# microsoft/MoGe

Measured on AMD Instinct MI355X. Metric: images/sec (MoGeModel.infer, moge-2-vitl 518x518 fp16), higher is better.
Workload: dtype f16; 1 GPU; moge-2-vitl infer(): batch 32/GPU x 3x518x518 torch.rand, num_tokens 3600, fp16 weights, synthetic checkpoint (seed 0), inputs resident in HBM, outputs left on device; global_batch=32, parallelism=dp1 (independent shards, one-time RCCL weight broadcast)

## Files before the change

moge_amd/csrc/attention_pp.hip:

```cpp
#include "common.h"

#define AP_GPTR(p) ((const __attribute__((address_space(1))) void*)(p))
#define AP_LPTR(p) ((__attribute__((address_space(3))) void*)(p))

typedef short s16x4 __attribute__((ext_vector_type(4)));

__device__ __forceinline__ u32x4 tr_pair(const char* p0, const char* p1) {
    const s16x4 a = __builtin_amdgcn_ds_read_tr16_b64_v4i16((__attribute__((address_space(3))) s16x4*)(p0));
    const s16x4 b = __builtin_amdgcn_ds_read_tr16_b64_v4i16((__attribute__((address_space(3))) s16x4*)(p1));
    typedef short s16x8 __attribute__((ext_vector_type(8)));
    const s16x8 v = {a[0], a[1], a[2], a[3], b[0], b[1], b[2], b[3]};
    return __builtin_bit_cast(u32x4, v);
}

__device__ __forceinline__ u32x4 pack8(const f32x16& p, int s) {
    f16x8 h;
#pragma unroll
    for (int i = 0; i < 8; i++) h[i] = (f16)p[8 * s + i];
    return __builtin_bit_cast(u32x4, h);
}

constexpr int AP_STAGE = 16384;
constexpr float AP_PSUM_LIMIT = 16384.f;

#ifdef MOGE_EXPERIMENTS
#include "../../tools/experiments/attention_pp_exp.inc"
#endif

constexpr int AP_VAR_DEFAULT = 0;
constexpr int AP_X_DEFAULT = 0;
constexpr int AP_KERN_DEFAULT = 3;
constexpr float AP_SCORE_LIMIT = 15.f;
constexpr float AP_ROWSUM_LIMIT = 49152.f;
template <int VAR>
__global__ __launch_bounds__(256, 3) void attn_pp16_kernel(const f16* __restrict__ q, const f16* __restrict__ k, const f16* __restrict__ v,
                                                           f16* __restrict__ out, int Ntok, int nh) {
    constexpr int NW = 4, NPW = 4;
    extern __shared__ __attribute__((aligned(16))) char smem[];

    const int tid = threadIdx.x, lane = tid & 63;
    const int wave = __builtin_amdgcn_readfirstlane(tid >> 6);
    const int l15 = lane & 15, g4 = lane >> 4;
    const int bh = blockIdx.y;
    const int b = bh / nh, head = bh - b * nh;
    const int q0 = blockIdx.x * (NW * 32) + wave * 32;

    u32x4 qf[2][2];
#pragma unroll
    for (int qb = 0; qb < 2; qb++) {
        const int qrow = q0 + qb * 16 + l15;
        const f16* qp = q + ((size_t)bh * Ntok + (qrow < Ntok ? qrow : Ntok - 1)) * 64;
#pragma unroll
        for (int ks = 0; ks < 2; ks++) qf[qb][ks] = *reinterpret_cast<const u32x4*>(qp + 32 * ks + 8 * g4);
    }

    const char* kbase = reinterpret_cast<const char*>(k + (size_t)bh * Ntok * 64);
    const char* vbase = reinterpret_cast<const char*>(v + (size_t)bh * Ntok * 64);
    const int prow = lane >> 3, pch = lane & 7;
    int drow[NPW];
    unsigned doff[NPW];
#pragma unroll
    for (int i = 0; i < NPW; i++) {
        const int p = wave + NW * i;
        const int row = (p & 7) * 8 + prow;
        drow[i] = row;
        const int ksw = ((row >> 1) & 1) | (((row >> 3) & 3) << 1);
        const int vsw = (((row >> 1) & 1) << 1) | (((row >> 3) & 1) << 2);
        doff[i] = (unsigned)(row * 128 + ((pch ^ (p >= 8 ? vsw : ksw)) << 4));
    }
    const int ntiles = (Ntok + 63) >> 6;
    auto issue = [&](int t) {
        char* st = smem + (t % 3) * AP_STAGE;
        const char* kt = uniform_ptr(kbase + (size_t)t * 8192);
        const char* vt = uniform_ptr(vbase + (size_t)t * 8192);
        if (t < ntiles - 1) {
#pragma unroll
            for (int i = 0; i < NPW; i++) {
                const int p = wave + NW * i;
                __builtin_amdgcn_global_load_lds(AP_GPTR((p >= 8 ? vt : kt) + doff[i]), AP_LPTR(st + p * 1024), 16, 0, 0);
            }
        } else {
#pragma unroll
            for (int i = 0; i < NPW; i++) {
                const int p = wave + NW * i;
                const int over = t * 64 + drow[i] - (Ntok - 1);
                const unsigned off = doff[i] - (over > 0 ? (unsigned)over * 128u : 0u);
                __builtin_amdgcn_global_load_lds(AP_GPTR((p >= 8 ? vt : kt) + off), AP_LPTR(st + p * 1024), 16, 0, 0);
            }
        }
    };

    const int kswl = ((l15 >> 1) & 1) | ((l15 >> 2) << 1);
    int kaddr[2];
#pragma unroll
    for (int ks = 0; ks < 2; ks++) kaddr[ks] = (8 * (l15 >> 2) + (l15 & 3)) * 128 + (((4 * ks + g4) ^ kswl) << 4);
    const int vswl = (((l15 >> 3) & 1) << 1) | ((g4 & 1) << 2);
    int vaddr[4];
#pragma unroll
    for (int db = 0; db < 4; db++)
        vaddr[db] = 8192 + (8 * g4 + (l15 >> 2)) * 128 + ((((2 * db) ^ vswl) | ((l15 & 3) >> 1)) << 4) + (l15 & 1) * 8;

    f32x4 o[4][2];
    f32x4 negs[2];
    float m_run[2], l_run[2];
#pragma unroll
    for (int qb = 0; qb < 2; qb++) {
#pragma unroll
        for (int db = 0; db < 4; db++) o[db][qb] = f32x4{0.f, 0.f, 0.f, 0.f};
        negs[qb] = f32x4{0.f, 0.f, 0.f, 0.f};
        m_run[qb] = -1e30f; l_run[qb] = 0.f;
    }

    issue(0);
    if (ntiles > 1) issue(1);

    int stage = 0;
    const char* ka[2];
    const char* va[4];
    f32x4 sc[4][2];
    float psum[2];
    auto tile_head = [&](int t) {
        if (t + 1 < ntiles) asm volatile("s_waitcnt vmcnt(%0)" ::"n"(NPW) : "memory");
        else asm volatile("s_waitcnt vmcnt(0)" ::: "memory");
        __builtin_amdgcn_s_barrier();
        asm volatile("" ::: "memory");
        if (t + 2 < ntiles) issue(t + 2);
        const int so = stage * AP_STAGE;
        stage = stage == 2 ? 0 : stage + 1;
#pragma unroll
        for (int ks = 0; ks < 2; ks++) ka[ks] = smem + (kaddr[ks] + so);
#pragma unroll
        for (int db = 0; db < 4; db++) va[db] = smem + (vaddr[db] + so);
    };
    auto pv = [&]() {
#pragma unroll
        for (int qb = 0; qb < 2; qb++) l_run[qb] += psum[qb];
#pragma unroll
        for (int s2 = 0; s2 < 2; s2++) {
            u32x4 pf[2];
#pragma unroll
            for (int qb = 0; qb < 2; qb++) {
                f16x8 hp;
#pragma unroll
                for (int r = 0; r < 4; r++) { hp[r] = (f16)sc[2 * s2][qb][r]; hp[4 + r] = (f16)sc[2 * s2 + 1][qb][r]; }
                pf[qb] = __builtin_bit_cast(u32x4, hp);
            }
#pragma unroll
            for (int db = 0; db < 4; db++) {
                const u32x4 vf = tr_pair(va[db] + (32 * ((VAR & 32) ? 0 : s2)) * 128, va[db] + (32 * ((VAR & 32) ? 0 : s2) + 4) * 128);
#pragma unroll
                for (int qb = 0; qb < 2; qb++) mma16<f16>(o[db][qb], vf, pf[qb]);
            }
        }
    };
    auto exact_body = [&](int t, bool last) {
#pragma unroll
        for (int kb = 0; kb < 4; kb++) {
            const int koff = (32 * (kb >> 1) + 4 * (kb & 1)) * 128;
            const u32x4 kf0 = *reinterpret_cast<const u32x4*>(ka[0] + koff), kf1 = *reinterpret_cast<const u32x4*>(ka[1] + koff);
#pragma unroll
            for (int qb = 0; qb < 2; qb++) {
                sc[kb][qb] = f32x4{0.f, 0.f, 0.f, 0.f};
                mma16<f16>(sc[kb][qb], kf0, qf[qb][0]);
                mma16<f16>(sc[kb][qb], kf1, qf[qb][1]);
            }
        }
#pragma unroll
        for (int qb = 0; qb < 2; qb++) {
            if (last) {
#pragma unroll
                for (int kb = 0; kb < 4; kb++)
#pragma unroll
                    for (int r = 0; r < 4; r++) {
                        const int key = t * 64 + 32 * (kb >> 1) + 8 * g4 + 4 * (kb & 1) + r;
                        if (key >= Ntok) sc[kb][qb][r] = -1e30f;
                    }
            }
            float mx = sc[0][qb][0];
#pragma unroll
            for (int kb = 0; kb < 4; kb++)
#pragma unroll
                for (int r = 0; r < 4; r++) mx = fmaxf(mx, sc[kb][qb][r]);
            mx = fmaxf(mx, __shfl_xor(mx, 16));
            mx = fmaxf(mx, __shfl_xor(mx, 32));
            const float m_new = fmaxf(m_run[qb], mx);
            const float alpha = __builtin_amdgcn_exp2f(m_run[qb] - m_new);
            m_run[qb] = m_new;
            l_run[qb] *= alpha;
#pragma unroll
            for (int db = 0; db < 4; db++)
#pragma unroll
                for (int r = 0; r < 4; r++) o[db][qb][r] *= alpha;
#pragma unroll
            for (int r = 0; r < 4; r++) negs[qb][r] = -m_new;
            float ps = 0.f;
#pragma unroll
            for (int kb = 0; kb < 4; kb++)
#pragma unroll
                for (int r = 0; r < 4; r++) {
                    sc[kb][qb][r] = __builtin_amdgcn_exp2f(sc[kb][qb][r] - m_new);
                    ps += sc[kb][qb][r];
                }
            psum[qb] = ps;
        }
        pv();
    };

    tile_head(0);
    exact_body(0, ntiles == 1);
    int t = 1;
    for (;;) {
        bool hit = false;
        for (; t < ntiles - 1; t++) {
            tile_head(t);
            if constexpr (VAR & 4) {
                u32x4 kf[4][2];
#pragma unroll
                for (int kb = 0; kb < 4; kb++) {
                    const int koff = (32 * (kb >> 1) + 4 * (kb & 1)) * 128;
                    kf[kb][0] = *reinterpret_cast<const u32x4*>(ka[0] + koff);
                    kf[kb][1] = *reinterpret_cast<const u32x4*>(ka[1] + koff);
                }
#pragma unroll
                for (int kb = 0; kb < 4; kb++)
#pragma unroll
                    for (int qb = 0; qb < 2; qb++)
                        sc[kb][qb] = __builtin_amdgcn_mfma_f32_16x16x32_f16(__builtin_bit_cast(f16x8, kf[kb][0]), __builtin_bit_cast(f16x8, qf[qb][0]), negs[qb], 0, 0, 0);
#pragma unroll
                for (int kb = 0; kb < 4; kb++)
#pragma unroll
                    for (int qb = 0; qb < 2; qb++) mma16<f16>(sc[kb][qb], kf[kb][1], qf[qb][1]);
            } else {
#pragma unroll
            for (int kb = 0; kb < 4; kb++) {
                const int koff = (32 * (kb >> 1) + 4 * (kb & 1)) * 128;
                const u32x4 kf0 = *reinterpret_cast<const u32x4*>(ka[0] + koff), kf1 = *reinterpret_cast<const u32x4*>(ka[1] + koff);
#pragma unroll
                for (int qb = 0; qb < 2; qb++) {
                    sc[kb][qb] = __builtin_amdgcn_mfma_f32_16x16x32_f16(__builtin_bit_cast(f16x8, kf0), __builtin_bit_cast(f16x8, qf[qb][0]), negs[qb], 0, 0, 0);
                    mma16<f16>(sc[kb][qb], kf1, qf[qb][1]);
                }
            }
            }
            bool trig = false;
            if constexpr ((VAR & 8) != 0) {
                float mx = sc[0][0][0];
#pragma unroll
                for (int kb = 0; kb < 4; kb++)
#pragma unroll
                    for (int qb = 0; qb < 2; qb++)
#pragma unroll
                        for (int r = 0; r < 4; r++) mx = fmaxf(mx, sc[kb][qb][r]);
                trig = !(mx <= AP_SCORE_LIMIT);
                if (__builtin_expect(__any(trig), 0)) { hit = true; break; }
            }
#pragma unroll
            for (int qb = 0; qb < 2; qb++) {
                float ps0 = 0.f, ps1 = 0.f;
#pragma unroll
                for (int kb = 0; kb < 4; kb++)
#pragma unroll
                    for (int r = 0; r < 4; r++) {
                        sc[kb][qb][r] = (VAR & 1) ? sc[kb][qb][r] * 1e-3f : __builtin_amdgcn_exp2f(sc[kb][qb][r]);
                        if (!(VAR & 16) || (kb == 0 && r == 0)) { if (kb & 1) ps1 += sc[kb][qb][r]; else ps0 += sc[kb][qb][r]; }
                    }
                psum[qb] = ps0 + ps1;
                trig |= !(psum[qb] < AP_PSUM_LIMIT);
            }
            if constexpr ((VAR & (2 | 8)) == 0) {
                if (__builtin_expect(__any(trig), 0)) { hit = true; break; }
            }
            pv();
        }
        if (!hit) break;
        exact_body(t, false);
        t++;
    }
    if (ntiles > 1) {
        tile_head(ntiles - 1);
        exact_body(ntiles - 1, true);
    }
#pragma unroll
    for (int qb = 0; qb < 2; qb++) {
        float l_tot = l_run[qb] + __shfl_xor(l_run[qb], 16);
        l_tot += __shfl_xor(l_tot, 32);
        const float inv = 1.f / l_tot;
        const int qrow = q0 + qb * 16 + l15;
        if (qrow < Ntok) {
            f16* op = out + ((size_t)b * Ntok + qrow) * ((size_t)nh * 64) + head * 64;
#pragma unroll
            for (int db = 0; db < 4; db++)
                store4(op + 16 * db + 4 * g4, o[db][qb][0] * inv, o[db][qb][1] * inv, o[db][qb][2] * inv, o[db][qb][3] * inv);
        }
    }
}

template <int QB> struct AttnAcc { f32x4 o[4][QB]; float m[QB], l[QB]; };
template <int QB, bool SK = false>
__device__ __forceinline__ bool attn_pp16mq_body(const f16* __restrict__ q, const f16* __restrict__ k, const f16* __restrict__ v, f16* __restrict__ out,
                                                 int Ntok, int nh, int bh, int q_base, char* smem, int tb_in = 0, int te_in = 0, AttnAcc<QB>* acc = nullptr,
                                                 const char* seed_k = nullptr) {
    constexpr int NW = 4, NPW = 4;
    const int tid = threadIdx.x, lane = tid & 63;
    const int wave = __builtin_amdgcn_readfirstlane(tid >> 6) & (NW - 1);
    const int l15 = lane & 15, g4 = lane >> 4;
    const int b = bh / nh, head = bh - b * nh;
    const int q0 = q_base + wave * (16 * QB);
    u32x4 qf[QB][2];
#pragma unroll
    for (int qb = 0; qb < QB; qb++) {
        const int qrow = q0 + qb * 16 + l15;
        const f16* qp = q + ((size_t)bh * Ntok + (qrow < Ntok ? qrow : Ntok - 1)) * 64;
#pragma unroll
        for (int ks = 0; ks < 2; ks++) qf[qb][ks] = *reinterpret_cast<const u32x4*>(qp + 32 * ks + 8 * g4);
    }
    const char* kbase = reinterpret_cast<const char*>(k + (size_t)bh * Ntok * 64);
    const char* vbase = reinterpret_cast<const char*>(v + (size_t)bh * Ntok * 64);
    const int prow = lane >> 3, pch = lane & 7;
    unsigned doff[NPW], doff_last[NPW];
    const int ntiles = (Ntok + 63) >> 6;
    const int tb = SK ? tb_in : 0, te = SK ? te_in : ntiles;
#pragma unroll
    for (int i = 0; i < NPW; i++) {
        const int p = wave + NW * i;
        const int row = (p & 7) * 8 + prow;
        const int ksw = ((row >> 1) & 1) | (((row >> 3) & 3) << 1);
        const int vsw = (((row >> 1) & 1) << 1) | (((row >> 3) & 1) << 2);
        doff[i] = (unsigned)(row * 128 + ((pch ^ (p >= 8 ? vsw : ksw)) << 4));
        const int over = (ntiles - 1) * 64 + row - (Ntok - 1);
        doff_last[i] = doff[i] - (over > 0 ? (unsigned)over * 128u : 0u);
    }
    auto issue = [&](int t) {
        char* st = smem + ((SK ? t - tb : t) % 3) * AP_STAGE;
        const char* kt = uniform_ptr(kbase + (size_t)t * 8192);
        const char* vt = uniform_ptr(vbase + (size_t)t * 8192);
        const bool last = t >= ntiles - 1;
#pragma unroll
        for (int i = 0; i < NPW; i++) {
            const int p = wave + NW * i;
            __builtin_amdgcn_global_load_lds(AP_GPTR((p >= 8 ? vt : kt) + (last ? doff_last[i] : doff[i])), AP_LPTR(st + p * 1024), 16, 0, 0);
        }
    };
    const int kswl = ((l15 >> 1) & 1) | ((l15 >> 2) << 1);
    int kaddr[2];
#pragma unroll
    for (int ks = 0; ks < 2; ks++) kaddr[ks] = (8 * (l15 >> 2) + (l15 & 3)) * 128 + (((4 * ks + g4) ^ kswl) << 4);
    const int vswl = (((l15 >> 3) & 1) << 1) | ((g4 & 1) << 2);
    int vaddr[4];
#pragma unroll
    for (int db = 0; db < 4; db++)
        vaddr[db] = 8192 + (8 * g4 + (l15 >> 2)) * 128 + ((((2 * db) ^ vswl) | ((l15 & 3) >> 1)) << 4) + (l15 & 1) * 8;

    f32x4 o[4][QB];
    f32x4 negs[QB];
    float m_run[QB], l_run[QB];
#pragma unroll
    for (int qb = 0; qb < QB; qb++) {
#pragma unroll
        for (int db = 0; db < 4; db++) o[db][qb] = f32x4{0.f, 0.f, 0.f, 0.f};
        negs[qb] = f32x4{0.f, 0.f, 0.f, 0.f};
        m_run[qb] = -1e30f; l_run[qb] = 0.f;
    }
    issue(tb);
    if (te - tb > 1) issue(tb + 1);

    int stage = 0;
    const char* ka[2];
    const char* va[4];
    f32x4 sc[4][QB];
    float psum[QB];
    auto tile_head = [&](int t, bool with_issue = true) {
        if (t + 1 < te) asm volatile("s_waitcnt vmcnt(%0)" ::"n"(NPW) : "memory");
        else asm volatile("s_waitcnt vmcnt(0)" ::: "memory");
        __builtin_amdgcn_s_barrier();
        asm volatile("" ::: "memory");
        if (with_issue && t + 2 < te) issue(t + 2);
        const int so = stage * AP_STAGE;
        stage = stage == 2 ? 0 : stage + 1;
#pragma unroll
        for (int ks = 0; ks < 2; ks++) ka[ks] = smem + (kaddr[ks] + so);
#pragma unroll
        for (int db = 0; db < 4; db++) va[db] = smem + (vaddr[db] + so);
    };
    auto pack = [&](int qb, u32x4 (&pf)[2]) {
#pragma unroll
        for (int s2 = 0; s2 < 2; s2++) {
            f16x8 hp;
#pragma unroll
            for (int r = 0; r < 4; r++) { hp[r] = (f16)sc[2 * s2][qb][r]; hp[4 + r] = (f16)sc[2 * s2 + 1][qb][r]; }
            pf[s2] = __builtin_bit_cast(u32x4, hp);
        }
    };
    auto pv_block = [&](int qb, const u32x4 (&pf)[2]) {
        l_run[qb] += psum[qb];
#pragma unroll
        for (int s2 = 0; s2 < 2; s2++)
#pragma unroll
            for (int db = 0; db < 4; db++) {
                const u32x4 vf = tr_pair(va[db] + (32 * s2) * 128, va[db] + (32 * s2 + 4) * 128);
                mma16<f16>(o[db][qb], vf, pf[s2]);
            }
    };
    auto exact_block = [&](int t, bool last, int qb) {
#pragma unroll
        for (int kb = 0; kb < 4; kb++) {
            const int koff = (32 * (kb >> 1) + 4 * (kb & 1)) * 128;
            const u32x4 kf0 = *reinterpret_cast<const u32x4*>(ka[0] + koff), kf1 = *reinterpret_cast<const u32x4*>(ka[1] + koff);
            sc[kb][qb] = f32x4{0.f, 0.f, 0.f, 0.f};
            mma16<f16>(sc[kb][qb], kf0, qf[qb][0]);
            mma16<f16>(sc[kb][qb], kf1, qf[qb][1]);
        }
        if (last) {
#pragma unroll
            for (int kb = 0; kb < 4; kb++)
#pragma unroll
                for (int r = 0; r < 4; r++) {
                    const int key = t * 64 + 32 * (kb >> 1) + 8 * g4 + 4 * (kb & 1) + r;
                    if (key >= Ntok) sc[kb][qb][r] = -1e30f;
                }
        }
        float mx = sc[0][qb][0];
#pragma unroll
        for (int kb = 0; kb < 4; kb++)
#pragma unroll
            for (int r = 0; r < 4; r++) mx = fmaxf(mx, sc[kb][qb][r]);
        mx = fmaxf(mx, __shfl_xor(mx, 16));
        mx = fmaxf(mx, __shfl_xor(mx, 32));
        const float m_new = fmaxf(m_run[qb], mx);
        const float alpha = __builtin_amdgcn_exp2f(m_run[qb] - m_new);
        m_run[qb] = m_new;
        l_run[qb] *= alpha;
#pragma unroll
        for (int db = 0; db < 4; db++)
#pragma unroll
            for (int r = 0; r < 4; r++) o[db][qb][r] *= alpha;
#pragma unroll
        for (int r = 0; r < 4; r++) negs[qb][r] = -m_new;
        float ps = 0.f;
#pragma unroll
        for (int kb = 0; kb < 4; kb++)
#pragma unroll
            for (int r = 0; r < 4; r++) {
                sc[kb][qb][r] = __builtin_amdgcn_exp2f(sc[kb][qb][r] - m_new);
                ps += sc[kb][qb][r];
            }
        ps += __shfl_xor(ps, 16);
        ps += __shfl_xor(ps, 32);
        psum[qb] = ps;
        u32x4 pf[2];
        pack(qb, pf);
        pv_block(qb, pf);
    };
    auto qk_block = [&](int qb, const u32x4 (&kf)[4][2]) {
#pragma unroll
        for (int kb = 0; kb < 4; kb++)
            sc[kb][qb] = __builtin_amdgcn_mfma_f32_16x16x32_f16(__builtin_bit_cast(f16x8, kf[kb][0]), __builtin_bit_cast(f16x8, qf[qb][0]), negs[qb], 0, 0, 0);
#pragma unroll
        for (int kb = 0; kb < 4; kb++) mma16<f16>(sc[kb][qb], kf[kb][1], qf[qb][1]);
    };
    u32x4 ones;
#pragma unroll
    for (int i = 0; i < 4; i++) ones[i] = 0x3c003c00u;
    const f32x4 zero4 = {0.f, 0.f, 0.f, 0.f};

    if (__builtin_amdgcn_readfirstlane(q0) >= Ntok) {
        for (int tt = tb; tt < te; tt++) tile_head(tt);
        return false;
    }
    bool seeded = false;
    if constexpr (SK) seeded = seed_k != nullptr && tb < ntiles - 1;
    tile_head(tb, !seeded);
    if constexpr (SK) if (seed_k) {
#pragma unroll
        for (int qb = 0; qb < QB; qb++) {
            float mx = -1e30f;
#pragma unroll
            for (int kb = 0; kb < 4; kb++) {
                const int koff = (32 * (kb >> 1) + 4 * (kb & 1)) * 128;
                const u32x4 kf0 = *reinterpret_cast<const u32x4*>(seed_k + kaddr[0] + koff), kf1 = *reinterpret_cast<const u32x4*>(seed_k + kaddr[1] + koff);
                f32x4 s0 = {0.f, 0.f, 0.f, 0.f};
                mma16<f16>(s0, kf0, qf[qb][0]);
                mma16<f16>(s0, kf1, qf[qb][1]);
#pragma unroll
                for (int r = 0; r < 4; r++) mx = fmaxf(mx, s0[r]);
            }
            mx = fmaxf(mx, __shfl_xor(mx, 16));
            mx = fmaxf(mx, __shfl_xor(mx, 32));
            m_run[qb] = mx;
#pragma unroll
            for (int r = 0; r < 4; r++) negs[qb][r] = -mx;
        }
    }
    int t = tb + 1;
    if (seeded) t = tb;
    else {
#pragma unroll
        for (int qb = 0; qb < QB; qb++) exact_block(tb, tb == ntiles - 1, qb);
    }
    const int hot_end = SK ? (te < ntiles - 1 ? te : ntiles - 1) : ntiles - 1;
    u32x4 pf[QB][2];
    f32x4 lt[QB];
    for (;;) {
        bool hit = false;
        for (; t < hot_end; t++) {
            if (!(seeded && t == tb)) tile_head(t, false);
            u32x4 kf[4][2];
#pragma unroll
            for (int kb = 0; kb < 4; kb++) {
                const int koff = (32 * (kb >> 1) + 4 * (kb & 1)) * 128;
                kf[kb][0] = *reinterpret_cast<const u32x4*>(ka[0] + koff);
                kf[kb][1] = *reinterpret_cast<const u32x4*>(ka[1] + koff);
            }
            __builtin_amdgcn_sched_barrier(0);
            if (t + 2 < te) issue(t + 2);
            __builtin_amdgcn_sched_barrier(0);
#pragma unroll
            for (int qb = 0; qb < QB; qb++) qk_block(qb, kf);
#pragma unroll
            for (int qb = 0; qb < QB; qb++) {
#pragma unroll
                for (int kb = 0; kb < 4; kb++)
#pragma unroll
                    for (int r = 0; r < 4; r++) sc[kb][qb][r] = __builtin_amdgcn_exp2f(sc[kb][qb][r]);
                pack(qb, pf[qb]);
                lt[qb] = __builtin_amdgcn_mfma_f32_16x16x32_f16(__builtin_bit_cast(f16x8, ones), __builtin_bit_cast(f16x8, pf[qb][0]), zero4, 0, 0, 0);
                mma16<f16>(lt[qb], ones, pf[qb][1]);
            }
            bool trig = false;
#pragma unroll
            for (int qb = 0; qb < QB; qb++) trig |= !(lt[qb][0] < AP_ROWSUM_LIMIT);
            if (__builtin_expect(__any(trig), 0)) { hit = true; break; }
#pragma unroll
            for (int qb = 0; qb < QB; qb++) l_run[qb] += lt[qb][0];
            {
                constexpr int AHEAD = QB == 4 ? 5 : 4;
                u32x4 vf[8];
                auto ld = [&](int gi) { vf[gi] = tr_pair(va[gi & 3] + (32 * (gi >> 2)) * 128, va[gi & 3] + (32 * (gi >> 2) + 4) * 128); };
#pragma unroll
                for (int gi = 0; gi < AHEAD; gi++) ld(gi);
                __builtin_amdgcn_sched_barrier(0);
#pragma unroll
                for (int gi = 0; gi < 8; gi++) {
                    if (gi + AHEAD < 8) ld(gi + AHEAD);
#pragma unroll
                    for (int qb = 0; qb < QB; qb++) mma16<f16>(o[gi & 3][qb], vf[gi], pf[qb][gi >> 2]);
                    __builtin_amdgcn_sched_barrier(0);
                }
            }
        }
        if (!hit) break;
#pragma unroll
        for (int qb = 0; qb < QB; qb++) {
            if (__any(!(lt[qb][0] < AP_ROWSUM_LIMIT))) exact_block(t, false, qb);
            else { psum[qb] = lt[qb][0]; pv_block(qb, pf[qb]); }
        }
        t++;
    }
    if (SK ? (te == ntiles && ntiles - 1 > tb) : (ntiles > 1)) {
        tile_head(ntiles - 1);
#pragma unroll
        for (int qb = 0; qb < QB; qb++) exact_block(ntiles - 1, true, qb);
    }
    if constexpr (SK) {
#pragma unroll
        for (int qb = 0; qb < QB; qb++) {
#pragma unroll
            for (int db = 0; db < 4; db++) acc->o[db][qb] = o[db][qb];
            acc->m[qb] = m_run[qb]; acc->l[qb] = l_run[qb];
        }
        return true;
    }
#pragma unroll
    for (int qb = 0; qb < QB; qb++) {
        const float inv = 1.f / l_run[qb];
        const int qrow = q0 + qb * 16 + l15;
        if (qrow < Ntok) {
            f16* op = out + ((size_t)b * Ntok + qrow) * ((size_t)nh * 64) + head * 64;
#pragma unroll
            for (int db = 0; db < 4; db++)
                store4(op + 16 * db + 4 * g4, o[db][qb][0] * inv, o[db][qb][1] * inv, o[db][qb][2] * inv, o[db][qb][3] * inv);
        }
    }
    return true;
}

template <int QB>
__global__ __launch_bounds__(256, QB > 2 ? 2 : 3) void attn_pp16mq_kernel(const f16* __restrict__ q, const f16* __restrict__ k, const f16* __restrict__ v,
                                                            f16* __restrict__ out, int Ntok, int nh, int xcd_remap, int q_start) {
    extern __shared__ __attribute__((aligned(16))) char smem[];
    int bh = blockIdx.y, qblk = blockIdx.x;
    if (((gridDim.y & 7) == 0) && (xcd_remap & 1)) {
        const int lin = blockIdx.y * gridDim.x + blockIdx.x;
        const int x = lin & 7, s = lin >> 3;
        const int hs = s / (int)gridDim.x;
        bh = x + 8 * hs;
        qblk = s - hs * (int)gridDim.x;
    }
    const int q_base = q_start + qblk * (64 * QB);
    if constexpr (QB == 4) if (xcd_remap & 2) {
        if (Ntok - q_base <= 128) { attn_pp16mq_body<2>(q, k, v, out, Ntok, nh, bh, q_base, smem); return; }
    }
    attn_pp16mq_body<QB>(q, k, v, out, Ntok, nh, bh, q_base, smem);
}

constexpr int AP_KS_MIN_TILES = 8;
template <int QB>
__global__ __launch_bounds__(512, 1) void attn_pp16ks_kernel(const f16* __restrict__ q, const f16* __restrict__ k, const f16* __restrict__ v,
                                                            f16* __restrict__ out, int Ntok, int nh, int xcd_remap, int tmid) {
    extern __shared__ __attribute__((aligned(16))) char smem[];
    int bh = blockIdx.y, qblk = blockIdx.x;
    if (((gridDim.y & 7) == 0) && (xcd_remap & 1)) {
        const int lin = blockIdx.y * gridDim.x + blockIdx.x;
        const int x = lin & 7, s = lin >> 3;
        const int hs = s / (int)gridDim.x;
        bh = x + 8 * hs;
        qblk = s - hs * (int)gridDim.x;
    }
    const int q_base = qblk * (64 * QB);
    const int tid = threadIdx.x, lane = tid & 63, t4 = tid & 255;
    const int wave8 = __builtin_amdgcn_readfirstlane(tid >> 6), grp = wave8 >> 2, wave = wave8 & 3;
    const int ntiles = (Ntok + 63) >> 6;
    AttnAcc<QB> a;
    const bool active = attn_pp16mq_body<QB, true>(q, k, v, out, Ntok, nh, bh, q_base, smem + grp * (3 * AP_STAGE), grp ? tmid : 0, grp ? ntiles : tmid, &a, grp ? smem : nullptr);
    for (int i = grp ? ntiles - tmid : tmid, n = max(tmid, ntiles - tmid); i < n; i++) __builtin_amdgcn_s_barrier();
    __syncthreads();
    f32x4* ex_o = reinterpret_cast<f32x4*>(smem);
    f32x2* ex_ml = reinterpret_cast<f32x2*>(smem + (size_t)4 * QB * 256 * 16);
    if (grp && active) {
#pragma unroll
        for (int db = 0; db < 4; db++)
#pragma unroll
            for (int qb = 0; qb < QB; qb++) ex_o[(db * QB + qb) * 256 + t4] = a.o[db][qb];
#pragma unroll
        for (int qb = 0; qb < QB; qb++) ex_ml[qb * 256 + t4] = f32x2{a.m[qb], a.l[qb]};
    }
    __syncthreads();
    if (grp || !active) return;
    const int l15 = lane & 15, g4 = lane >> 4;
    const int b = bh / nh, head = bh - b * nh;
    const int q0 = q_base + wave * (16 * QB);
#pragma unroll
    for (int qb = 0; qb < QB; qb++) {
        const f32x2 ml = ex_ml[qb * 256 + t4];
        const float mstar = fmaxf(a.m[qb], ml[0]);
        const float w0 = __builtin_amdgcn_exp2f(a.m[qb] - mstar), w1 = __builtin_amdgcn_exp2f(ml[0] - mstar);
        const float l = fmaf(w1, ml[1], w0 * a.l[qb]);
        const float inv = 1.f / l;
        const int qrow = q0 + qb * 16 + l15;
#pragma unroll
        for (int db = 0; db < 4; db++) {
            const f32x4 o1 = ex_o[(db * QB + qb) * 256 + t4];
            f32x4 o;
#pragma unroll
            for (int r = 0; r < 4; r++) o[r] = fmaf(w1, o1[r], w0 * a.o[db][qb][r]);
            if (qrow < Ntok) {
                f16* op = out + ((size_t)b * Ntok + qrow) * ((size_t)nh * 64) + head * 64;
                store4(op + 16 * db + 4 * g4, o[0] * inv, o[1] * inv, o[2] * inv, o[3] * inv);
            }
        }
    }
}

#ifdef MOGE_EXPERIMENTS
#include "../../tools/experiments/attention_pp16sk_exp.inc"
#else
size_t attention_pp_ws_bytes(int, int, int) { return 0; }
size_t attention_pp_ws_counter_bytes(int, int, int) { return 0; }
#endif

#ifdef MOGE_EXPERIMENTS
#include "../../tools/experiments/attention_pp16s_exp.inc"
#include "../../tools/experiments/attention_pp16x_exp.inc"
#endif


static int launch_attn_pp16(const void* q, const void* k, const void* v, void* out, int B, int nh, int Ntok, hipStream_t st, void* ws, size_t ws_bytes) {
    constexpr int smem = 3 * AP_STAGE;
#ifdef MOGE_EXPERIMENTS
    {
        int QB, nx, gx;
        if (ws && attn_sk_plan(B, nh, Ntok, &QB, &nx, &gx) && ws_bytes >= attention_pp_ws_bytes(B, nh, Ntok)) {
            int* cnt = reinterpret_cast<int*>(ws);
            float* part = reinterpret_cast<float*>(reinterpret_cast<char*>(ws) + attention_pp_ws_counter_bytes(B, nh, Ntok));
            if (QB == 4) {
                if (int rc = set_dyn_lds<attn_pp16sk_kernel<4>>(smem)) return rc;
                hipLaunchKernelGGL(attn_pp16sk_kernel<4>, dim3(nx * gx), dim3(256), smem, st, (const f16*)q, (const f16*)k, (const f16*)v, (f16*)out, Ntok, nh, nx, B * nh / nx, part, cnt);
            } else {
                if (int rc = set_dyn_lds<attn_pp16sk_kernel<2>>(smem)) return rc;
                hipLaunchKernelGGL(attn_pp16sk_kernel<2>, dim3(nx * gx), dim3(256), smem, st, (const f16*)q, (const f16*)k, (const f16*)v, (f16*)out, Ntok, nh, nx, B * nh / nx, part, cnt);
            }
            return (int)hipGetLastError();
        }
    }
#else
    (void)ws; (void)ws_bytes;
#endif
    dim3 grid((Ntok + 127) / 128, B * nh);
    const int akern = moge_tune_get("ATTN_KERN", AP_KERN_DEFAULT);
    if (akern >= 1) {
        const long wgs2 = (long)((Ntok + 127) / 128) * B * nh;
        const bool q4 = akern == 2 || akern == 4 || (akern == 3 && wgs2 > moge_tune_get("ATTN_Q2_MAX_WGS", 3 * pp_device_cus()));
        const int xr = (moge_tune_get("ATTN_XCD", 1) ? 1 : 0) | (moge_tune_get("ATTN_TAIL2", 1) ? 2 : 0);
#ifdef MOGE_EXPERIMENTS
        const int nfull = Ntok / 512, rem = Ntok - nfull * 512;
        const int nblk = nfull + (rem > 256 ? 1 : 0);
        const bool xk = nblk > 0 && (akern == 4 || (akern == 3 && moge_tune_get("ATTN_X", AP_X_DEFAULT) &&
                                                    (long)nblk * B * nh >= (long)moge_tune_get("ATTN_X_MIN_ROUNDS", 2) * pp_device_cus()));
        if (xk) {
            constexpr int smem_x = 4 * AP_STAGE + 8 * 8192;
            if (moge_tune_get("ATTN_X_TS", 0)) {
                static unsigned long long* dts = nullptr;
                if (!dts && hipMalloc(&dts, 16 * sizeof(unsigned long long)) != hipSuccess) return -1;
                (void)hipMemsetAsync(dts, 0, 16 * sizeof(unsigned long long), st);
                if (int rc = set_dyn_lds<attn_pp16x_kernel<0, 1>>(smem_x)) return rc;
                hipLaunchKernelGGL((attn_pp16x_kernel<0, 1>), dim3(nblk, B * nh), dim3(512), smem_x, st, (const f16*)q, (const f16*)k, (const f16*)v, (f16*)out, Ntok, nh, xr, dts);
                unsigned long long h[16];
                (void)hipMemcpyAsync(h, dts, sizeof(h), hipMemcpyDeviceToHost, st);
                (void)hipStreamSynchronize(st);
                for (int g2 = 0; g2 < 2; g2++)
                    if (h[g2 * 8 + 4])
                        fprintf(stderr, "[attn_pp16x ts] group %d: %llu hot tiles; per tile (s_memtime ticks): E body %.0f, barrier wait %.0f, M body %.0f, barrier wait %.0f\n", g2, h[g2 * 8 + 4],
                                (double)h[g2 * 8 + 0] / h[g2 * 8 + 4], (double)h[g2 * 8 + 1] / h[g2 * 8 + 4], (double)h[g2 * 8 + 2] / h[g2 * 8 + 4], (double)h[g2 * 8 + 3] / h[g2 * 8 + 4]);
            } else if (moge_tune_get("ATTN_X_PRIO", 0)) {
                if (int rc = set_dyn_lds<attn_pp16x_kernel<1>>(smem_x)) return rc;
                hipLaunchKernelGGL(attn_pp16x_kernel<1>, dim3(nblk, B * nh), dim3(512), smem_x, st, (const f16*)q, (const f16*)k, (const f16*)v, (f16*)out, Ntok, nh, xr);
            } else {
                if (int rc = set_dyn_lds<attn_pp16x_kernel<0>>(smem_x)) return rc;
                hipLaunchKernelGGL(attn_pp16x_kernel<0>, dim3(nblk, B * nh), dim3(512), smem_x, st, (const f16*)q, (const f16*)k, (const f16*)v, (f16*)out, Ntok, nh, xr);
            }
            const int covered = nblk * 512;
            if (covered < Ntok) {
                if (int rc = set_dyn_lds<attn_pp16mq_kernel<4>>(smem)) return rc;
                hipLaunchKernelGGL(attn_pp16mq_kernel<4>, dim3((Ntok - covered + 255) / 256, B * nh), dim3(256), smem, st, (const f16*)q, (const f16*)k, (const f16*)v, (f16*)out, Ntok, nh, xr, covered);
            }
            return (int)hipGetLastError();
        }
#endif
#ifdef MOGE_EXPERIMENTS
        const int sfull = Ntok / 256;
        if ((akern == 6 || akern == 7) && sfull > 0 && Ntok > 128) {
            constexpr int smem_s = APS_NSTG * AP_STAGE + 4 * 8192;
            if (akern == 6) {
                if (int rc = set_dyn_lds<attn_pp16s_kernel<1>>(smem_s)) return rc;
                hipLaunchKernelGGL(attn_pp16s_kernel<1>, dim3(sfull, B * nh), dim3(256), smem_s, st, (const f16*)q, (const f16*)k, (const f16*)v, (f16*)out, Ntok, nh, xr);
            } else {
                constexpr int smem_s2 = 5 * AP_STAGE;
                if (int rc = set_dyn_lds<attn_pp16s_kernel<2>>(smem_s2)) return rc;
                hipLaunchKernelGGL(attn_pp16s_kernel<2>, dim3(sfull, B * nh), dim3(256), smem_s2, st, (const f16*)q, (const f16*)k, (const f16*)v, (f16*)out, Ntok, nh, xr);
            }
            const int covered = sfull * 256;
            if (covered < Ntok) {
                if (int rc = set_dyn_lds<attn_pp16mq_kernel<4>>(smem)) return rc;
                hipLaunchKernelGGL(attn_pp16mq_kernel<4>, dim3((Ntok - covered + 255) / 256, B * nh), dim3(256), smem, st, (const f16*)q, (const f16*)k, (const f16*)v, (f16*)out, Ntok, nh, xr, covered);
            }
            return (int)hipGetLastError();
        }
#endif
        if (const int ks = moge_tune_get("ATTN_KS", 1); ks > 1 || (ks == 1 && akern == 3)) {
            constexpr int smem_ks = 6 * AP_STAGE;
            const int cus = pp_device_cus(), ntiles = (Ntok + 63) >> 6;
            const long w2 = (long)((Ntok + 127) / 128) * B * nh, w4 = (long)((Ntok + 255) / 256) * B * nh;
            const bool fits = ks == 1 && ntiles >= AP_KS_MIN_TILES;
            int tmid = (ntiles + 1) >> 1;
            if (const int f = moge_tune_get("ATTN_KS_MID", 0); f > 0 && f < ntiles) tmid = f;
            if ((ks == 2 && ntiles >= 2) || (fits && w2 <= cus)) {
                if (int rc = set_dyn_lds<attn_pp16ks_kernel<2>>(smem_ks)) return rc;
                hipLaunchKernelGGL(attn_pp16ks_kernel<2>, dim3((Ntok + 127) / 128, B * nh), dim3(512), smem_ks, st, (const f16*)q, (const f16*)k, (const f16*)v, (f16*)out, Ntok, nh, xr, tmid);
                return (int)hipGetLastError();
            }
            if ((ks == 4 && ntiles >= 2) || (fits && w4 <= cus)) {
                if (int rc = set_dyn_lds<attn_pp16ks_kernel<4>>(smem_ks)) return rc;
                hipLaunchKernelGGL(attn_pp16ks_kernel<4>, dim3((Ntok + 255) / 256, B * nh), dim3(512), smem_ks, st, (const f16*)q, (const f16*)k, (const f16*)v, (f16*)out, Ntok, nh, xr, tmid);
                return (int)hipGetLastError();
            }
        }
        if (q4) {
            if (int rc = set_dyn_lds<attn_pp16mq_kernel<4>>(smem)) return rc;
            hipLaunchKernelGGL(attn_pp16mq_kernel<4>, dim3((Ntok + 255) / 256, B * nh), dim3(256), smem, st, (const f16*)q, (const f16*)k, (const f16*)v, (f16*)out, Ntok, nh, xr, 0);
        } else {
            if (int rc = set_dyn_lds<attn_pp16mq_kernel<2>>(smem)) return rc;
            hipLaunchKernelGGL(attn_pp16mq_kernel<2>, grid, dim3(256), smem, st, (const f16*)q, (const f16*)k, (const f16*)v, (f16*)out, Ntok, nh, xr, 0);
        }
        return (int)hipGetLastError();
    }
#define AP_LAUNCH_VAR(V) do { if (int rc = set_dyn_lds<attn_pp16_kernel<V>>(smem)) return rc; \
        hipLaunchKernelGGL(attn_pp16_kernel<V>, grid, dim3(256), smem, st, (const f16*)q, (const f16*)k, (const f16*)v, (f16*)out, Ntok, nh); \
        return (int)hipGetLastError(); } while (0)
#ifdef MOGE_EXPERIMENTS
    switch (moge_tune_get("ATTN_VAR", AP_VAR_DEFAULT)) {
    case 0: AP_LAUNCH_VAR(0);
    case 1: AP_LAUNCH_VAR(1);
    case 2: AP_LAUNCH_VAR(2);
    case 4: AP_LAUNCH_VAR(4);
    case 6: AP_LAUNCH_VAR(6);
    case 8: AP_LAUNCH_VAR(8);
    case 12: AP_LAUNCH_VAR(12);
    case 16: AP_LAUNCH_VAR(16);
    case 18: AP_LAUNCH_VAR(18);
    case 19: AP_LAUNCH_VAR(19);
    case 32: AP_LAUNCH_VAR(32);
    case 50: AP_LAUNCH_VAR(50);
    case 51: AP_LAUNCH_VAR(51);
    default: return -1;
    }
#else
    AP_LAUNCH_VAR(AP_VAR_DEFAULT);
#endif
#undef AP_LAUNCH_VAR
}

#ifdef MOGE_EXPERIMENTS
template <int NW, int QT>
static int launch_attn_pp_cfg(const void* q, const void* k, const void* v, void* out, int B, int nh, int Ntok, hipStream_t st) {
    constexpr int smem = 3 * AP_STAGE;
    constexpr auto kern = attn_pp_kernel<NW, QT>;
    if (int rc = set_dyn_lds<kern>(smem)) return rc;
    dim3 grid((Ntok + NW * 32 * QT - 1) / (NW * 32 * QT), B * nh);
    hipLaunchKernelGGL(kern, grid, dim3(NW * 64), smem, st, (const f16*)q, (const f16*)k, (const f16*)v, (f16*)out, Ntok, nh);
    return (int)hipGetLastError();
}
#endif

int launch_attention_pp(const void* q, const void* k, const void* v, void* out, int B, int nh, int Ntok, hipStream_t st, void* ws, size_t ws_bytes) {
    if (Ntok < 1) return -1;
#ifdef MOGE_EXPERIMENTS
    switch (moge_tune_get("ATTN_EXP", 0)) {
    case 1: return launch_attn_pp_cfg<4, 1>(q, k, v, out, B, nh, Ntok, st);
    case 2: return launch_attn_pp_cfg<4, 2>(q, k, v, out, B, nh, Ntok, st);
    case 3: return launch_attn_pp_cfg<8, 1>(q, k, v, out, B, nh, Ntok, st);
    default: break;
    }
#endif
    return launch_attn_pp16(q, k, v, out, B, nh, Ntok, st, ws, ws_bytes);
}
```

Baseline: 249.8 images/s.

## Trim half-empty last key tile, add QB=1 tail path, schedule tail blocks last

When the last key tile is at most half full, the QK and PV MFMAs for its empty half are skipped and those scores are masked. Query tail blocks with 32 or fewer rows now use a single-query-block body. The XCD block remap can place tail query blocks at the end of the grid so they fill in after the full blocks. All three are on by default through tune flags. In exchange, the kernel gains extra branches and template instantiations.

```diff
diff --git a/moge_amd/csrc/attention_pp.hip b/moge_amd/csrc/attention_pp.hip
--- a/moge_amd/csrc/attention_pp.hip
+++ b/moge_amd/csrc/attention_pp.hip
@@ -299,7 +299,7 @@
 template <int QB, bool SK = false>
 __device__ __forceinline__ bool attn_pp16mq_body(const f16* __restrict__ q, const f16* __restrict__ k, const f16* __restrict__ v, f16* __restrict__ out,
                                                  int Ntok, int nh, int bh, int q_base, char* smem, int tb_in = 0, int te_in = 0, AttnAcc<QB>* acc = nullptr,
-                                                 const char* seed_k = nullptr) {
+                                                 const char* seed_k = nullptr, bool trim = false) {
     constexpr int NW = 4, NPW = 4;
     const int tid = threadIdx.x, lane = tid & 63;
     const int wave = __builtin_amdgcn_readfirstlane(tid >> 6) & (NW - 1);
@@ -391,19 +391,21 @@
             pf[s2] = __builtin_bit_cast(u32x4, hp);
         }
     };
-    auto pv_block = [&](int qb, const u32x4 (&pf)[2]) {
+    auto pv_block = [&](int qb, const u32x4 (&pf)[2], bool half = false) {
         l_run[qb] += psum[qb];
 #pragma unroll
         for (int s2 = 0; s2 < 2; s2++)
 #pragma unroll
             for (int db = 0; db < 4; db++) {
+                if (s2 == 1 && half) break;
                 const u32x4 vf = tr_pair(va[db] + (32 * s2) * 128, va[db] + (32 * s2 + 4) * 128);
                 mma16<f16>(o[db][qb], vf, pf[s2]);
             }
     };
-    auto exact_block = [&](int t, bool last, int qb) {
+    auto exact_block = [&](int t, bool last, int qb, bool half = false) {
 #pragma unroll
         for (int kb = 0; kb < 4; kb++) {
+            if (kb >= 2 && half) { sc[kb][qb] = f32x4{-1e30f, -1e30f, -1e30f, -1e30f}; continue; }
             const int koff = (32 * (kb >> 1) + 4 * (kb & 1)) * 128;
             const u32x4 kf0 = *reinterpret_cast<const u32x4*>(ka[0] + koff), kf1 = *reinterpret_cast<const u32x4*>(ka[1] + koff);
             sc[kb][qb] = f32x4{0.f, 0.f, 0.f, 0.f};
@@ -438,18 +440,20 @@
         for (int r = 0; r < 4; r++) negs[qb][r] = -m_new;
         float ps = 0.f;
 #pragma unroll
-        for (int kb = 0; kb < 4; kb++)
+        for (int kb = 0; kb < 4; kb++) {
+            if (kb >= 2 && half) { sc[kb][qb] = f32x4{0.f, 0.f, 0.f, 0.f}; continue; }
 #pragma unroll
             for (int r = 0; r < 4; r++) {
                 sc[kb][qb][r] = __builtin_amdgcn_exp2f(sc[kb][qb][r] - m_new);
                 ps += sc[kb][qb][r];
             }
+        }
         ps += __shfl_xor(ps, 16);
         ps += __shfl_xor(ps, 32);
         psum[qb] = ps;
         u32x4 pf[2];
         pack(qb, pf);
-        pv_block(qb, pf);
+        pv_block(qb, pf, half);
     };
     auto qk_block = [&](int qb, const u32x4 (&kf)[4][2]) {
 #pragma unroll
@@ -558,8 +562,9 @@
     }
     if (SK ? (te == ntiles && ntiles - 1 > tb) : (ntiles > 1)) {
         tile_head(ntiles - 1);
-#pragma unroll
-        for (int qb = 0; qb < QB; qb++) exact_block(ntiles - 1, true, qb);
+        const bool half = trim && (ntiles - 1) * 64 + 32 >= Ntok;
+#pragma unroll
+        for (int qb = 0; qb < QB; qb++) exact_block(ntiles - 1, true, qb, half);
     }
     if constexpr (SK) {
 #pragma unroll
@@ -582,6 +587,18 @@
         }
     }
     return true;
+}
+
+__host__ __device__ inline void attn_pp_block_map(int lin, int gx, int gy, bool tails_last, int* bh, int* qblk) {
+    const int x = lin & 7, s = lin >> 3;
+    int hs = s / gx, qb = s - hs * gx;
+    if (tails_last && gx > 1) {
+        const int nfull = gx - 1, body = (gy >> 3) * nfull;
+        if (s < body) { hs = s / nfull; qb = s - hs * nfull; }
+        else { hs = s - body; qb = nfull; }
+    }
+    *bh = x + 8 * hs;
+    *qblk = qb;
 }
 
 template <int QB>
@@ -590,17 +607,17 @@
     extern __shared__ __attribute__((aligned(16))) char smem[];
     int bh = blockIdx.y, qblk = blockIdx.x;
     if (((gridDim.y & 7) == 0) && (xcd_remap & 1)) {
-        const int lin = blockIdx.y * gridDim.x + blockIdx.x;
-        const int x = lin & 7, s = lin >> 3;
-        const int hs = s / (int)gridDim.x;
-        bh = x + 8 * hs;
-        qblk = s - hs * (int)gridDim.x;
+        const int rem = Ntok - q_start - ((int)gridDim.x - 1) * (64 * QB);
+        attn_pp_block_map(blockIdx.y * gridDim.x + blockIdx.x, (int)gridDim.x, (int)gridDim.y, (xcd_remap & 8) && rem <= 32 * QB, &bh, &qblk);
     }
     const int q_base = q_start + qblk * (64 * QB);
-    if constexpr (QB == 4) if (xcd_remap & 2) {
-        if (Ntok - q_base <= 128) { attn_pp16mq_body<2>(q, k, v, out, Ntok, nh, bh, q_base, smem); return; }
-    }
-    attn_pp16mq_body<QB>(q, k, v, out, Ntok, nh, bh, q_base, smem);
+    const bool trim = (xcd_remap & 4) != 0;
+    if constexpr (QB == 4) {
+        const int left = Ntok - q_base;
+        if ((xcd_remap & 16) && left <= 32) { attn_pp16mq_body<1>(q, k, v, out, Ntok, nh, bh, q_base, smem, 0, 0, nullptr, nullptr, trim); return; }
+        if ((xcd_remap & 2) && left <= 128) { attn_pp16mq_body<2>(q, k, v, out, Ntok, nh, bh, q_base, smem, 0, 0, nullptr, nullptr, trim); return; }
+    }
+    attn_pp16mq_body<QB>(q, k, v, out, Ntok, nh, bh, q_base, smem, 0, 0, nullptr, nullptr, trim);
 }
 
 constexpr int AP_KS_MIN_TILES = 8;
@@ -700,7 +717,8 @@
     if (akern >= 1) {
         const long wgs2 = (long)((Ntok + 127) / 128) * B * nh;
         const bool q4 = akern == 2 || akern == 4 || (akern == 3 && wgs2 > moge_tune_get("ATTN_Q2_MAX_WGS", 3 * pp_device_cus()));
-        const int xr = (moge_tune_get("ATTN_XCD", 1) ? 1 : 0) | (moge_tune_get("ATTN_TAIL2", 1) ? 2 : 0);
+        const int xr = (moge_tune_get("ATTN_XCD", 1) ? 1 : 0) | (moge_tune_get("ATTN_TAIL2", 1) ? 2 : 0) | (moge_tune_get("ATTN_LTRIM", 1) ? 4 : 0) |
+                       (moge_tune_get("ATTN_TAILLAST", 1) ? 8 : 0) | (moge_tune_get("ATTN_TAIL1", 1) ? 16 : 0);
 #ifdef MOGE_EXPERIMENTS
         const int nfull = Ntok / 512, rem = Ntok - nfull * 512;
         const int nblk = nfull + (rem > 256 ? 1 : 0);
@@ -775,8 +793,12 @@
             }
         }
         if (q4) {
+            int gx4 = (Ntok + 255) / 256;
+#ifdef MOGE_EXPERIMENTS
+            if (moge_tune_get("ATTN_KB_NOTAIL", 0) && Ntok >= 256) gx4 = Ntok / 256;
+#endif
             if (int rc = set_dyn_lds<attn_pp16mq_kernel<4>>(smem)) return rc;
-            hipLaunchKernelGGL(attn_pp16mq_kernel<4>, dim3((Ntok + 255) / 256, B * nh), dim3(256), smem, st, (const f16*)q, (const f16*)k, (const f16*)v, (f16*)out, Ntok, nh, xr, 0);
+            hipLaunchKernelGGL(attn_pp16mq_kernel<4>, dim3(gx4, B * nh), dim3(256), smem, st, (const f16*)q, (const f16*)k, (const f16*)v, (f16*)out, Ntok, nh, xr, 0);
         } else {
             if (int rc = set_dyn_lds<attn_pp16mq_kernel<2>>(smem)) return rc;
             hipLaunchKernelGGL(attn_pp16mq_kernel<2>, grid, dim3(256), smem, st, (const f16*)q, (const f16*)k, (const f16*)v, (f16*)out, Ntok, nh, xr, 0);
```

Result: no change. 251.9 images/s (median of 6 runs) (+0.9%).
